# Penguin77jp/RaytracingMin

Measured on AMD Instinct MI355X. Metric: Msamples/s (W*H*spp/s), Cornell box 1080p@1024spp, higher is better.
Workload: dtype f64; 1 GPU; cornellBoxSetting.json rows 0:1080 of 1920x1080 1024spp (SS 4 x S 64), L1 repaired, max_bounces 8, seed 0x5EED, host-libm sin/cos (RTM_MODE_HOST_TRIG), interleaved 8-row bands over 1 GPU(s) + one gather; sample_split_waves_per_tile=8, collective=none (one rank, frame stays in HBM)

## Files before the change

### include/rtm_debug.h

```cpp
#ifndef RTM_DEBUG_H
#define RTM_DEBUG_H

#include "rtm.h"

#ifdef __cplusplus
extern "C" {
#endif

int rtm_debug_math_probe(int op, const double* a, const double* b, size_t n, double* out);
int rtm_debug_trig_table(int entries, double* out);
int rtm_debug_selfcheck(int kind, unsigned long long* mismatches);
int rtm_debug_wf_nearest(int kind, const rtm_sphere* spheres, size_t n, const double* org, const double* dir,
                         size_t n_rays, int32_t* out_id, double* out_t);
int rtm_debug_fp64_peak(int waves_per_simd, double min_ms, double* tflops, double* kernel_ms);
int rtm_debug_grid_nearest(const rtm_sphere* spheres, size_t n, const double* org, const double* dir, size_t n_rays,
                           int32_t* out_id, double* out_t, uint32_t* out_tests, uint32_t* out_steps, uint64_t* info);
int rtm_debug_grid_build(const rtm_sphere* spheres, size_t n, uint64_t* info, double* pads, uint32_t* ranges, size_t ranges_cap,
                         uint32_t* items, size_t items_cap, int32_t* big, size_t big_cap);
int rtm_debug_scene_facts(const rtm_sphere* spheres, size_t n, uint64_t facts[2]);
int rtm_debug_zero_term_facts(const rtm_sphere* spheres, size_t n, uint64_t facts[2]);
int rtm_debug_component_bench(int which, const rtm_sphere* spheres, size_t n, int reps, int blocks, int lds_pad,
                              double* cycles_per_rep);
int rtm_debug_denoise_variance_kernel(int form, const rtm_denoise_var_params* params, int32_t width, int32_t height, int device,
                                      const rtm_aov_buffers* guide_dev, void* work_dev, float* variance_out_dev, void* stream);
int rtm_debug_matte_rank(int32_t super_samples, int32_t layers, int device, const int32_t* ids_dev, size_t n_pixels,
                         int32_t* id_out_dev, float* coverage_out_dev, float* alpha_out_dev, void* stream);

#ifdef __cplusplus
}
#endif
#endif
```

### raytracingmin_amd/_lib.py

```python
import ctypes as C
import os

_HERE = os.path.dirname(os.path.abspath(__file__))
LIB_PATH = os.environ.get("RTM_LIB_OVERRIDE") or os.path.join(_HERE, "librtm_hip.so")

RTM_OK = 0
MODE_LITERAL, MODE_REPAIRED = 0, 1
MODE_HOST_TRIG = 0x100
MODE_COUNT_TESTS = 0x200
MODE_SURFACE_SAMPLE = 0x400
MODES = {"literal": MODE_LITERAL, "repaired": MODE_REPAIRED, 0: 0, 1: 1}


class RtmError(RuntimeError):
    def __init__(self, status, what, detail=""):
        self.status = status
        super().__init__(f"{what}: {detail}" if detail else what)


class rtm_camera(C.Structure):
    _fields_ = [("origin", C.c_double * 3), ("target", C.c_double * 3), ("up", C.c_double * 3),
                ("fov", C.c_float), ("_pad", C.c_float)]


# ... 175 lines not shown
    "rtm_scene_load_json_objects": (C.c_int, [C.c_char_p, C.c_int, _P(rtm_settings), C.c_void_p,
                                              C.c_size_t, _P(C.c_size_t)]),
    "rtm_scene_parse_json_objects": (C.c_int, [C.c_char_p, C.c_size_t, C.c_int, _P(rtm_settings),
                                               C.c_void_p, C.c_size_t, _P(C.c_size_t)]),
    "rtm_scene_save_sample_json": (C.c_int, [C.c_char_p]),
    "rtm_scene_make_stress": (C.c_int, [C.c_uint64, C.c_size_t, _P(rtm_settings), C.c_void_p]),
    "rtm_quantise": (C.c_int, [C.c_void_p, C.c_size_t, C.c_void_p]),
    "rtm_write_bmp": (C.c_int, [C.c_char_p, C.c_int, C.c_int, C.c_int, C.c_void_p]),
    "rtm_write_jpg": (C.c_int, [C.c_char_p, C.c_int, C.c_int, C.c_int, C.c_void_p, C.c_int]),
    "rtm_write_pfm": (C.c_int, [C.c_char_p, C.c_int, C.c_int, C.c_int, C.c_void_p]),
    "rtm_read_pfm": (C.c_int, [C.c_char_p, _P(C.c_int), _P(C.c_int), _P(C.c_int), C.c_void_p, C.c_size_t]),
}
DEBUG_SIGNATURES = {
    "rtm_debug_math_probe": (C.c_int, [C.c_int, C.c_void_p, C.c_void_p, C.c_size_t, C.c_void_p]),
    "rtm_debug_selfcheck": (C.c_int, [C.c_int, C.POINTER(C.c_uint64)]),
    "rtm_debug_trig_table": (C.c_int, [C.c_int, C.c_void_p]),
    "rtm_debug_fp64_peak": (C.c_int, [C.c_int, C.c_double, C.POINTER(C.c_double), C.POINTER(C.c_double)]),
    "rtm_debug_wf_nearest": (C.c_int, [C.c_int, C.c_void_p, C.c_size_t, C.c_void_p, C.c_void_p, C.c_size_t,
                                       C.c_void_p, C.c_void_p]),
    "rtm_debug_grid_nearest": (C.c_int, [C.c_void_p, C.c_size_t, C.c_void_p, C.c_void_p, C.c_size_t, C.c_void_p, C.c_void_p,
                                         C.c_void_p, C.c_void_p, C.c_void_p]),
    "rtm_debug_scene_facts": (C.c_int, [C.c_void_p, C.c_size_t, C.c_void_p]),
    "rtm_debug_zero_term_facts": (C.c_int, [C.c_void_p, C.c_size_t, C.c_void_p]),
    "rtm_debug_grid_build": (C.c_int, [C.c_void_p, C.c_size_t, C.c_void_p, C.c_void_p, C.c_void_p, C.c_size_t, C.c_void_p,
                                       C.c_size_t, C.c_void_p, C.c_size_t]),
    "rtm_debug_denoise_variance_kernel": (C.c_int, [C.c_int, _P(rtm_denoise_var_params), C.c_int32, C.c_int32, C.c_int,
                                                    _P(rtm_aov_buffers), C.c_void_p, C.c_void_p, C.c_void_p]),
    "rtm_debug_matte_rank": (C.c_int, [C.c_int32, C.c_int32, C.c_int, C.c_void_p, C.c_size_t, C.c_void_p, C.c_void_p, C.c_void_p,
                                       C.c_void_p]),
    "rtm_debug_component_bench": (C.c_int, [C.c_int, C.c_void_p, C.c_size_t, C.c_int, C.c_int, C.c_int,
                                            C.POINTER(C.c_double)]),
}
ABI_VERSION = 5

_lib = None


def _share_torch_hip_runtime():
    try:
        import torch
    except ImportError:
        pass


def lib():
    global _lib
# ... 23 lines not shown
```

### raytracingmin_amd/csrc/rtm_api.cpp

```cpp
#include <exception>

#include "../../include/rtm_debug.h"
#include "rtm_internal.h"

#define RTM_GUARD(call)                                  \
    try {                                                \
        return (call);                                   \
    } catch (const std::exception& e) {                  \
        rtm::set_last_error(e.what());                   \
        return RTM_ERR_INVALID_ARGUMENT;                 \
    } catch (...) {                                      \
        rtm::set_last_error("unknown exception");        \
        return RTM_ERR_INVALID_ARGUMENT;                 \
    }

extern "C" {

int rtm_abi_version(void) { return RTM_ABI_VERSION; }

const char* rtm_strerror(int status) {
    switch (status) {
        case RTM_OK: return "ok";
        case RTM_ERR_INVALID_ARGUMENT: return "invalid argument";
        case RTM_ERR_INVALID_SCENE: return "invalid scene";
// ... 166 lines not shown
    RTM_GUARD(rtm::wf_nearest_probe(kind, sp, n, org, dir, n_rays, out_id, out_t))
}
int rtm_debug_denoise_variance_kernel(int form, const rtm_denoise_var_params* params, int32_t width, int32_t height, int device,
                                      const rtm_aov_buffers* guide_dev, void* work_dev, float* variance_out_dev, void* stream) {
    RTM_GUARD(rtm::denoise_variance_kernel_probe(form, params, width, height, device, guide_dev, work_dev, variance_out_dev, stream))
}
int rtm_debug_matte_rank(int32_t super_samples, int32_t layers, int device, const int32_t* ids_dev, size_t n_pixels,
                         int32_t* id_out_dev, float* coverage_out_dev, float* alpha_out_dev, void* stream) {
    RTM_GUARD(rtm::matte_rank_probe(super_samples, layers, device, ids_dev, n_pixels, id_out_dev, coverage_out_dev, alpha_out_dev,
                                    stream))
}
int rtm_debug_trig_table(int entries, double* out) { RTM_GUARD(rtm::trig_table_host(entries, out)) }
int rtm_debug_selfcheck(int kind, unsigned long long* mismatches) { RTM_GUARD(rtm::selfcheck(kind, mismatches)) }
int rtm_debug_grid_nearest(const rtm_sphere* sp, size_t n, const double* org, const double* dir, size_t n_rays,
                           int32_t* out_id, double* out_t, uint32_t* out_tests, uint32_t* out_steps, uint64_t* info) {
    RTM_GUARD(rtm::grid_nearest_probe(sp, n, org, dir, n_rays, out_id, out_t, out_tests, out_steps, info))
}
int rtm_debug_grid_build(const rtm_sphere* sp, size_t n, uint64_t* info, double* pads, uint32_t* ranges, size_t ranges_cap,
                         uint32_t* items, size_t items_cap, int32_t* big, size_t big_cap) {
    RTM_GUARD(rtm::grid_build_host(sp, n, info, pads, ranges, ranges_cap, items, items_cap, big, big_cap))
}
int rtm_debug_scene_facts(const rtm_sphere* sp, size_t n, uint64_t facts[2]) { RTM_GUARD(rtm::scene_facts_host(sp, n, facts)) }
int rtm_debug_zero_term_facts(const rtm_sphere* sp, size_t n, uint64_t facts[2]) { RTM_GUARD(rtm::zero_term_facts_host(sp, n, facts)) }
int rtm_debug_fp64_peak(int waves_per_simd, double min_ms, double* tflops, double* kernel_ms) {
    RTM_GUARD(rtm::fp64_peak(waves_per_simd, min_ms, tflops, kernel_ms))
}

int rtm_scene_load_json(const char* path, int literal_loader, rtm_settings* settings,
                        rtm_sphere* spheres, size_t capacity, size_t* n_spheres) {
    RTM_GUARD(rtm::scene_load_json(path, literal_loader, settings, spheres, capacity, n_spheres))
}
int rtm_scene_parse_json(const char* text, size_t len, int literal_loader, rtm_settings* settings,
                         rtm_sphere* spheres, size_t capacity, size_t* n_spheres) {
    RTM_GUARD(rtm::scene_parse_json(text, len, literal_loader, settings, spheres, capacity, n_spheres))
}
int rtm_scene_save_sample_json(const char* path) { RTM_GUARD(rtm::scene_save_sample_json(path)) }
int rtm_scene_make_stress(uint64_t seed, size_t n, rtm_settings* settings, rtm_sphere* spheres) {
    RTM_GUARD(rtm::scene_make_stress(seed, n, settings, spheres))
}
int rtm_quantise(const double* image, size_t n_values, uint8_t* out) {
    RTM_GUARD(rtm::quantise(image, n_values, out))
}
int rtm_write_bmp(const char* filename, int w, int h, int comp, const void* data) {
    try {
        return rtm::write_bmp(filename, w, h, comp, data);
    } catch (...) {
// ... 27 lines not shown
```

### raytracingmin_amd/csrc/rtm_internal.h

```cpp
#pragma once
#include <stddef.h>
#include <stdint.h>

#include <string>

#include "../../include/rtm.h"

namespace rtm {

void set_last_error(const std::string& s);
const char* last_error();

int device_count(int* count);
int num_variants();
int output_rows(const rtm_options* opt);
int release_scratch(int device);
int stream_release(int device, void* stream);
int wf_nearest_probe(int kind, const rtm_sphere* sp, size_t n, const double* org, const double* dir, size_t n_rays,
                     int32_t* out_id, double* out_t);
const char* variant_name(int v);
int scene_create(const rtm_sphere* sp, size_t n, int on_device, int device, rtm_scene** out);
int scene_create_objects(const rtm_object* objs, size_t n, int device, rtm_scene** out);
int intersect_objects_batch(const rtm_object* objs, const double* org, const double* dir, size_t n, int mode,
                            int32_t* out_hit, double* out_t, double* out_normal);
// ... 47 lines not shown
                  const rtm_options* opt, double* out64, float* out32, uint8_t* out8, void* stream,
                  rtm_stats* stats);
int render_host(const rtm_settings* st, const rtm_sphere* sp, size_t n, const rtm_options* opt,
                double* out64, float* out32, uint8_t* out8, rtm_stats* stats);
int render_host_objects(const rtm_settings* st, const rtm_object* objs, size_t n, const rtm_options* opt,
                        double* out64, float* out32, uint8_t* out8, rtm_stats* stats);
int path_trace_batch(const rtm_sphere* sp, size_t n, const rtm_options* opt, const double* org,
                     const double* dir, size_t n_rays, double* out, uint32_t* out_draws,
                     uint32_t* out_casts);
int surface_sample_batch(const rtm_sphere* sp, size_t n, const rtm_options* opt, const double* org, const double* dir,
                         size_t n_rays, double* out, uint32_t* out_draws, uint32_t* out_casts);
int intersect_batch(const rtm_sphere* sp, const double* org, const double* dir, size_t n, int mode,
                    int32_t* out_hit, double* out_t, double* out_normal);
int rng_batch(uint64_t seed, uint32_t pixel0, uint32_t n_pixels, uint32_t sample, uint32_t n_draws,
              double* out);
double rng_u01_host(uint64_t seed, uint32_t pixel, uint32_t sample, uint32_t index);
int component_bench(int which, const rtm_sphere* sp, size_t n, int reps, int blocks, int lds_pad,
                    double* cycles_per_rep);
int selfcheck(int kind, unsigned long long* mismatches);
int grid_nearest_probe(const rtm_sphere* sp, size_t n, const double* org, const double* dir, size_t n_rays, int32_t* out_id,
                       double* out_t, uint32_t* out_tests, uint32_t* out_steps, uint64_t* info);
int scene_facts_host(const rtm_sphere* sp, size_t n, uint64_t* facts);
int zero_term_facts_host(const rtm_sphere* sp, size_t n, uint64_t* facts);
int grid_build_host(const rtm_sphere* sp, size_t n, uint64_t* info, double* pads, uint32_t* ranges, size_t ranges_cap,
                    uint32_t* items, size_t items_cap, int32_t* big, size_t big_cap);
int fp64_peak(int waves_per_simd, double min_ms, double* tflops, double* kernel_ms);
int math_probe(int op, const double* a, const double* b, size_t n, double* out);
int launch_tol(const void* render_params, size_t params_bytes, unsigned grid, size_t lds_pad, void* stream);
int tol_math_probe(int op, const double* a_dev, const double* b_dev, size_t n, double* out_dev);
int trig_table_host(int entries, double* out);
void release_trig_tab(int device);

int scene_parse_json(const char* text, size_t len, int literal_loader, rtm_settings* st,
                     rtm_sphere* spheres, size_t capacity, size_t* n_spheres);
int scene_parse_json_objects(const char* text, size_t len, int literal_loader, rtm_settings* st,
                             rtm_object* objects, size_t capacity, size_t* n_objects);
int scene_load_json_objects(const char* path, int literal_loader, rtm_settings* st, rtm_object* objects,
                            size_t capacity, size_t* n_objects);
int scene_load_json(const char* path, int literal_loader, rtm_settings* st, rtm_sphere* spheres,
                    size_t capacity, size_t* n_spheres);
int scene_save_sample_json(const char* path);
int scene_make_stress(uint64_t seed, size_t n, rtm_settings* st, rtm_sphere* spheres);
int quantise(const double* image, size_t n_values, uint8_t* out);
int write_bmp(const char* filename, int w, int h, int comp, const void* data);
int write_jpg(const char* filename, int w, int h, int comp, const void* data, int quality);
int write_pfm(const char* filename, int w, int h, int comp, const float* data);
// ... 4 lines not shown
```

### raytracingmin_amd/csrc/rtm_kernels.hip

```cpp
#include <hip/hip_runtime.h>

#include <cfloat>
#include <cmath>
#include <cstdio>
#include <cstdlib>
#include <cstring>
#include <algorithm>
#include <atomic>
#include <thread>
#include <map>
#include <memory>
#include <mutex>
#include <shared_mutex>
#include <tuple>
#include <string>
#include <type_traits>
#include <vector>

#include "../../include/rtm.h"
#include "rtm_device.h"
#include "rtm_host.h"
#include "rtm_path.h"

#include "rtm_render_kernel.h"
// ... 48 lines not shown
        m = m < sp[i].color[2] ? sp[i].color[2] : m;
        const double kd = (double)(float)m;
        mat[i * 8 + 0] = sp[i].color[0] / kd;
        mat[i * 8 + 1] = sp[i].color[1] / kd;
        mat[i * 8 + 2] = sp[i].color[2] / kd;
        mat[i * 8 + 3] = sp[i].emission[0];
        mat[i * 8 + 4] = sp[i].emission[1];
        mat[i * 8 + 5] = sp[i].emission[2];
        mat[i * 8 + 6] = kd;
        mat[i * 8 + 7] = kd * 16777216.0;
    }
}

static uint64_t axis_pattern(const double* geom, size_t n) {
    uint64_t pat = 0;
    for (size_t i = 0; i < n && i < 32; ++i) {
        const double* g = geom + i * 4;
        if (!(std::isfinite(g[0]) && std::isfinite(g[1]) && std::isfinite(g[2])) || !(g[3] >= 0.0)) continue;
        const bool zx = g[0] == 0.0, zy = g[1] == 0.0, zz = g[2] == 0.0;
        const uint64_t a = (!zx && zy && zz) ? 1u : (zx && !zy && zz) ? 2u : (zx && zy && !zz) ? 3u : 0u;
        pat |= a << (2 * i);
    }
    return pat;
}

static unsigned compact_flag_of(const double* geom, size_t n) {
    for (size_t i = 0; i < n; ++i) {
        const double* g = geom + i * 4;
        const double reach = std::sqrt(g[0] * g[0] + g[1] * g[1] + g[2] * g[2]) + std::sqrt(std::fabs(g[3]));
        if (!(reach <= kCompactExtent)) return 0u;
    }
    return kSceneCompact;
}
static unsigned fold_flags_of(const double* mat, size_t n) {
    auto plain = [](double v) { return !std::signbit(v) && !std::isnan(v); };
    for (size_t i = 0; i < n; ++i) {
        const double* m = mat + i * 8;
        if (!(plain(m[3]) && plain(m[4]) && plain(m[5]))) return 0u;
        if (m[6] > 0.0) {
            if (!(m[3] == 0.0 && m[4] == 0.0 && m[5] == 0.0)) return 0u;
            if (!(plain(m[0]) && plain(m[1]) && plain(m[2]))) return 0u;
        }
    }
    return kFoldNoLevelEmission;
}
static unsigned zero_term_flags_of(const double* mat, size_t n, uint64_t* emit_mask) {
// ... 386 lines not shown
            ranges[c * 2] = B.cell_start[c];
            ranges[c * 2 + 1] = B.cell_start[c + 1];
        }
    if (items) std::memcpy(items, B.items.data(), B.refs * sizeof(unsigned));
    if (big && !B.big.empty()) std::memcpy(big, B.big.data(), B.big.size() * sizeof(int));
    return RTM_OK;
}

int scene_facts_host(const rtm_sphere* sp, size_t n, uint64_t* facts) {
    if ((!sp && n) || !facts) return RTM_ERR_INVALID_ARGUMENT;
    std::vector<double> hg, hm;
    flatten_scene(sp, n, hg, hm);
    facts[0] = axis_pattern(hg.data(), n);
    facts[1] = fold_flags_of(hm.data(), n) | compact_flag_of(hg.data(), n);
    return RTM_OK;
}
int zero_term_facts_host(const rtm_sphere* sp, size_t n, uint64_t* facts) {
    if ((!sp && n) || !facts) return RTM_ERR_INVALID_ARGUMENT;
    std::vector<double> hg, hm;
    flatten_scene(sp, n, hg, hm);
    facts[0] = zero_term_flags_of(hm.data(), n, &facts[1]) != 0u ? 1u : 0u;
    return RTM_OK;
}

static int build_scene_grid(rtm_scene& sc, const double* hg, const double* hm, size_t n, int device,
                            const double* plane_rows = nullptr) {
    GridBuild B;
    if (!make_grid(hg, n, B)) return RTM_OK;
    sc.grid_far_bounces = false;
    const double reach = std::sqrt(B.hdr.reach2);
    for (int i : B.big) {
        const bool diffuse = !hm || hm[(size_t)i * 8 + 6] > 0.0;
        if (hg[(size_t)i * 4 + 3] < 0.0) {
            if (!plane_rows) return RTM_OK;
            const double* pl = plane_rows + (size_t)i * 16;
            for (int c = 0; c < 4 && diffuse; ++c) {
                double d2 = 0.0;
                for (int k = 0; k < 3; ++k) {
                    const double p = pl[k] + ((c & 1) ? pl[6 + k] : -pl[6 + k]) + ((c & 2) ? pl[9 + k] : -pl[9 + k]);
                    d2 += (p - B.hdr.cb[k]) * (p - B.hdr.cb[k]);
                }
                if (!(std::sqrt(d2) <= reach)) sc.grid_far_bounces = true;
            }
            continue;
        }
        double d2 = 0.0;
// ... 25 lines not shown
    B.hdr.cell_range = reinterpret_cast<const uint2*>(base + off_cs);
    B.hdr.recs = reinterpret_cast<const double4*>(base + off_items);
    B.hdr.n_recs = (unsigned)B.items.size();
    B.hdr.big = reinterpret_cast<const int*>(base + off_big);
    RTM_HIP_CHECK(hipMemcpy(base, &B.hdr, sizeof B.hdr, hipMemcpyHostToDevice));
    RTM_HIP_CHECK(hipMemcpy(base + off_cs, ranges.data(), ranges.size() * sizeof(unsigned), hipMemcpyHostToDevice));
    RTM_HIP_CHECK(hipMemcpy(base + off_items, recs.data(), recs.size() * sizeof(double), hipMemcpyHostToDevice));
    if (!B.big.empty())
        RTM_HIP_CHECK(hipMemcpy(base + off_big, B.big.data(), B.big.size() * sizeof(int), hipMemcpyHostToDevice));
    sc.grid_hdr = B.hdr;
    sc.grid_cells = B.cell_start.size() - 1;
    sc.grid_refs = B.items.size();
    sc.grid_big = B.big.size();
    return RTM_OK;
}

static int scene_build_host(rtm_scene& sc, const rtm_sphere* sp, size_t n, int device, bool want_grid = true) {
    RTM_HIP_CHECK(hipSetDevice(device));
    sc.device = device;
    sc.n = n;
    std::vector<double> hg, hm, hs;
    flatten_scene(sp, n, hg, hm, &hs);
    sc.axis_pat = axis_pattern(hg.data(), n);
    sc.fold_flags = fold_flags_of(hm.data(), n) | compact_flag_of(hg.data(), n) | zero_term_flags_of(hm.data(), n, &sc.emit_mask);
    int rc = sc.geom.alloc_pooled((n ? n : 1) * 4 * sizeof(double), device);
    if (rc == RTM_OK) rc = sc.mat.alloc_pooled((n + 1) * 8 * sizeof(double), device);
    if (rc == RTM_OK) rc = sc.aux.alloc_pooled(scene_aux_doubles(n) * sizeof(double), device);
    if (rc == RTM_OK) rc = sc.surf.alloc_pooled(hs.size() * sizeof(double), device);
    if (rc != RTM_OK) return rc;
    RTM_HIP_CHECK(hipMemcpy(sc.surf.p, hs.data(), hs.size() * sizeof(double), hipMemcpyHostToDevice));
    if (n) RTM_HIP_CHECK(hipMemcpy(sc.geom.p, hg.data(), hg.size() * sizeof(double), hipMemcpyHostToDevice));
    RTM_HIP_CHECK(hipMemcpy(sc.mat.p, hm.data(), hm.size() * sizeof(double), hipMemcpyHostToDevice));
    rc = launch_scene_aux(sc.geom.as<double>(), n, sc.aux.as<double>(), nullptr);
    if (rc != RTM_OK) return rc;
    RTM_HIP_CHECK(hipStreamSynchronize(nullptr));
    return want_grid ? build_scene_grid(sc, hg.data(), hm.data(), n, device) : RTM_OK;
}
static int scene_build_device(rtm_scene& sc, const rtm_sphere* sp_dev, size_t n, int device) {
    RTM_HIP_CHECK(hipSetDevice(device));
    sc.device = device;
    sc.n = n;
    int rc = sc.geom.alloc_pooled((n ? n : 1) * 4 * sizeof(double), device);
    if (rc == RTM_OK) rc = sc.mat.alloc_pooled((n + 1) * 8 * sizeof(double), device);
    if (rc == RTM_OK) rc = sc.aux.alloc_pooled(scene_aux_doubles(n) * sizeof(double), device);
    if (rc == RTM_OK) rc = sc.surf.alloc_pooled((n ? n : 1) * 4 * sizeof(double), device);
    if (rc != RTM_OK) return rc;
    flatten_scene_kernel<<<(unsigned)((n + 1 + 255) / 256), 256>>>(sp_dev, n, sc.geom.as<double>(), sc.mat.as<double>(), sc.surf.as<double>());
    RTM_HIP_CHECK(hipGetLastError());
    rc = launch_scene_aux(sc.geom.as<double>(), n, sc.aux.as<double>(), nullptr);
    if (rc != RTM_OK) return rc;
    RTM_HIP_CHECK(hipStreamSynchronize(nullptr));
    if (n > 0 && n <= 32) {
        std::vector<double> rows(n * 4);
        RTM_HIP_CHECK(hipMemcpy(rows.data(), sc.geom.p, rows.size() * sizeof(double), hipMemcpyDeviceToHost));
        sc.axis_pat = axis_pattern(rows.data(), n);
        std::vector<double> mrows((n + 1) * 8);
        RTM_HIP_CHECK(hipMemcpy(mrows.data(), sc.mat.p, mrows.size() * sizeof(double), hipMemcpyDeviceToHost));
        sc.fold_flags = fold_flags_of(mrows.data(), n) | compact_flag_of(rows.data(), n) | zero_term_flags_of(mrows.data(), n, &sc.emit_mask);
    }
    if (n < kGridMinSpheres) return RTM_OK;
    std::vector<double> hg(n * 4);
    RTM_HIP_CHECK(hipMemcpy(hg.data(), sc.geom.p, hg.size() * sizeof(double), hipMemcpyDeviceToHost));
    std::vector<double> hm((n + 1) * 8);
    RTM_HIP_CHECK(hipMemcpy(hm.data(), sc.mat.p, hm.size() * sizeof(double), hipMemcpyDeviceToHost));
    return build_scene_grid(sc, hg.data(), hm.data(), n, device);
}

int scene_create(const rtm_sphere* sp, size_t n, int on_device, int device, rtm_scene** out) {
    if (!out || (!sp && n) || n > 0x7FFFFFFFull) return invalid("null argument or scene too large");
    *out = nullptr;
    std::unique_ptr<rtm_scene> sc(new rtm_scene);
    const int rc = on_device ? scene_build_device(*sc, sp, n, device) : scene_build_host(*sc, sp, n, device);
    if (rc != RTM_OK) return rc;
    *out = sc.release();
    return RTM_OK;
}
static void plane_row(const rtm_object& o, double row[16]) {
    using namespace host;
    const H3 pos = {o.position[0], o.position[1], o.position[2]};
    const H3 nrm = normalize(sub(H3{o.target[0], o.target[1], o.target[2]}, pos));
    const H3 rn = normalize(cross(nrm, H3{o.up[0], o.up[1], o.up[2]}));
// ... 2004 lines not shown
```

### raytracingmin_amd/csrc/rtm_kernels_tol.hip

```cpp
#define RTM_NS rtm_tol
#define RTM_TOL 1
#include <hip/hip_runtime.h>

#include <cmath>
#include <cstdlib>
#include <cstring>
#include <map>
#include <mutex>
#include <vector>

#include "rtm_internal.h"
#include "rtm_render_kernel.h"

namespace rtm_tol {

static bool compact_launch(const RenderParams& P) {
    const double cam = std::sqrt(P.cam_org.x * P.cam_org.x + P.cam_org.y * P.cam_org.y + P.cam_org.z * P.cam_org.z);
    return (P.scene.fold_flags & kSceneCompact) != 0u && cam <= kCompactExtent;
}

constexpr unsigned kTolCapped = kLdsTab | kPark | kPack8 | kDefer | kSteal;
constexpr unsigned kTolAny = kLdsTab | kPark | kDefer | kPackL;
constexpr int kTolWavesPerSimd = 4;

template <unsigned F>
static void launch_n(const RenderParams& P, unsigned grid, size_t lds_pad, hipStream_t stream) {
    constexpr int LDS_D = (F & kPackL) != 0 ? 0 : 16;
    unsigned unit_tab;
    render_lds_bytes<F, uint8_t, LDS_D>(P.scene.n, lds_pad, &unit_tab);
    const bool axis = P.mode == RTM_MODE_REPAIRED && unit_tab == 1u && compact_launch(P);
#define RTM_AXIS_CASE(k, sig)                                                                                    \
    if (P.scene.n == k && P.scene.axis_pat == sig && axis) {                                                     \
        launch_tiles<MathFast, F, axis_unroll(k, sig), uint8_t, LDS_D, kTolWavesPerSimd>(P, grid, lds_pad, stream); \
        return;                                                                                                  \
    }
    if constexpr ((F & kPackL) != 0) {
        RTM_AXIS_CASE(7, kAxisSigCornell7)
    } else {
        RTM_AXIS_SIGNATURES(RTM_AXIS_CASE)
        switch (P.scene.n) {
            case 3: launch_tiles<MathFast, F, -103, uint8_t, LDS_D, kTolWavesPerSimd>(P, grid, lds_pad, stream); return;
            case 5: launch_tiles<MathFast, F, -105, uint8_t, LDS_D, kTolWavesPerSimd>(P, grid, lds_pad, stream); return;
            case 7: launch_tiles<MathFast, F, -107, uint8_t, LDS_D, kTolWavesPerSimd>(P, grid, lds_pad, stream); return;
            default: break;
        }
    }
#undef RTM_AXIS_CASE
    if (P.scene.n < 8) launch_tiles<MathFast, F, -8, uint8_t, LDS_D, kTolWavesPerSimd>(P, grid, lds_pad, stream);
    else launch_tiles<MathFast, F, 8, uint8_t, LDS_D, kTolWavesPerSimd>(P, grid, lds_pad, stream);
}

template <unsigned F>
static void launch_row(const RenderParams& P, unsigned grid, size_t lds_pad, hipStream_t stream) {
    if (P.split > 1) {
        launch_n<F | kSplit>(P, P.split_first + P.n_tiles * P.split, lds_pad, stream);
        launch_split_finalize(P, stream);
    } else {
        launch_n<F>(P, grid, lds_pad, stream);
    }
    if constexpr ((F & kSteal) != 0) launch_steal_finalize(P, grid, stream);
}

__global__ void tol_math_probe_kernel(int op, const double* __restrict__ a, const double* __restrict__ b, size_t n,
                                      double* __restrict__ out, const double2* __restrict__ tab) {
    const size_t i = (size_t)blockIdx.x * blockDim.x + threadIdx.x;
    if (i >= n) return;
    const double x = a[i], y = b ? b[i] : 0.0;
    double r = 0.0, s, c;
    switch (op) {
        case 32: r = seq_sqrt(x); break;
        case 33: r = seq_quot(x, y, seq_rcp(y)); break;
        case 34: r = seq_rcp(x); break;
        case 35: r = x * y + 1.0; break;
        case 36: sincos_small(x, s, c); r = s; break;
        case 37: sincos_small(x, s, c); r = c; break;
        case 38: r = fold_step(d3(x, x, x), d3(y, y, y), d3(0.25, 0.25, 0.25)).y; break;
        case 39: sincos_turn24_k(TrigFromRegs{}, x, s, c); r = s; break;
        case 40: sincos_turn24_k(TrigFromRegs{}, x, s, c); r = c; break;
        case 41: {
            const double in[1] = {x};
            double out1[1];
            seq_sqrt_batch<1, true>(in, out1);
            r = out1[0];
            break;
        }
        case 42: sincos_turn24_tab_apply(sincos_turn24_tab_load(tab, (uint32_t)x), s, c); r = s; break;
        case 43: sincos_turn24_tab_apply(sincos_turn24_tab_load(tab, (uint32_t)x), s, c); r = c; break;
        case 44: { MathSpec m; r = m.sqrt64_unit(x); } break;
        case 45: {
// ... 147 lines not shown
```

### raytracingmin_amd/csrc/rtm_path.h

```cpp
#pragma once
#include <cfloat>
#include <type_traits>

#include "../../include/rtm.h"
#include "rtm_device.h"

namespace RTM_NS {


__device__ __forceinline__ double seq_rcp(const double y) {
    double r = __builtin_amdgcn_rcp(y);
    double e = __builtin_fma(-y, r, 1.0);
#if RTM_TOL
    return __builtin_fma(r, __builtin_fma(e, e, e), r);
#else
    r = __builtin_fma(r, e, r);
    e = __builtin_fma(-y, r, 1.0);
    return __builtin_fma(r, e, r);
#endif
}
__device__ __forceinline__ double seq_quot(const double x, const double y, const double r) {
#if RTM_TOL
    (void)y;
    return x * r;
// ... 439 lines not shown
    const double4* recs;
    const int* big;
};

struct SceneView {
    const double4* __restrict__ geom;
    const double* __restrict__ mat;
    int n;
    const double* __restrict__ wprime = nullptr;
    const double* __restrict__ bounds = nullptr;
    const float4* __restrict__ geom32 = nullptr;
    const float4* __restrict__ geom32s = nullptr;
    const uint32_t* __restrict__ trig_fix = nullptr;
    const double* __restrict__ plane = nullptr;
    const GridHeader* __restrict__ grid = nullptr;
    const double* __restrict__ surf = nullptr;
    unsigned long long axis_pat = 0ull;
    unsigned fold_flags = 0u;
    unsigned long long emit_mask = ~0ull;
};
constexpr unsigned kFoldNoLevelEmission = 1u;
constexpr unsigned kFoldZeroTermSkippable = 4u;
constexpr unsigned kSceneCompact = 2u;
constexpr double kCompactExtent = 1e7;

__device__ __forceinline__ bool plane_test(const double* __restrict__ pl, const D3 org, const D3 dir, double& t) {
    const D3 pos = d3(pl[0], pl[1], pl[2]), nrm = d3(pl[3], pl[4], pl[5]);
    const double dn = dot(nrm, dir);
    if (fabs(dn) < (double)FLT_EPSILON) return false;
    const double tt = dot(nrm, pos - org) / dn;
    if (!(tt > 0.001)) return false;
    const D3 d = (org + dir * tt) - pos;
    const D3 right = d3(pl[6], pl[7], pl[8]), upv = d3(pl[9], pl[10], pl[11]);
    if (fabs(dot(d, right)) > pl[12] || fabs(dot(d, upv)) > pl[13]) return false;
    t = tt;
    return true;
}

struct TrigFixWord {
    uint32_t word;
    int off;
};
__device__ __forceinline__ TrigFixWord trig_fix_load(const uint32_t* __restrict__ fix, const RngStream& rng) {
    const uint32_t k = mix32((rng.ctr - 2u * 0x9E3779B9u) ^ rng.k1) >> 9;
    return TrigFixWord{fix[k >> 3], (int)(k & 7u) * 4};
}
// ... 165 lines not shown
                best = m;
            }
            dis = best;
            hit_object = (int)((((uint32_t)__double2loint(best)) + 1u) & 7u) - 1;
            return;
        }
    }
    if (!PACKID && far == 0ull) {
#pragma unroll
        for (int k = 0; k < K; ++k) {
            const unsigned long long accept = __builtin_amdgcn_ballot_w64(t1v[k] < dis);
            hit_object = sel_index_mask(accept, i0 + k, hit_object);
            double m;
            asm("v_min_f64 %0, %1, %2" : "=v"(m) : "v"(dis), "v"(t1v[k]));
            dis = m;
        }
        return;
    }
#endif
#pragma unroll
    for (int k = 0; k < K; ++k) accept_update(b[k], sq[k], i0 + k, dis, hit_object);
}

struct AxisShared {
#if RTM_TOL
    double Pyz, Pxz, Pxy, Qyz, Qxz, Qxy;
#else
    double Px, Py, Pz, Pxy, Qx, Qy, Qz, Qxy;
#endif
    __device__ __forceinline__ AxisShared(const D3 org, const D3 dir) {
        const double px = org.x * dir.x, py = org.y * dir.y, pz = org.z * dir.z;
        const double qx = org.x * org.x, qy = org.y * org.y, qz = org.z * org.z;
#if RTM_TOL
        Pyz = py + pz; Pxz = px + pz; Pxy = px + py;
        Qyz = qy + qz; Qxz = qx + qz; Qxy = qx + qy;
#else
        Px = px; Py = py; Pz = pz; Pxy = px + py;
        Qx = qx; Qy = qy; Qz = qz; Qxy = qx + qy;
#endif
    }
};
constexpr unsigned kAxisSigCornell7 = 2u | (1u << 2) | (1u << 4) | (2u << 6) | (2u << 8) | (3u << 10) | (3u << 12);
constexpr unsigned kAxisSigSimple5 = (1u << 2) | (1u << 4) | (2u << 6) | (2u << 8);
constexpr unsigned kAxisSigSetting3 = 2u | (1u << 4);
constexpr int axis_unroll(const int n, const unsigned sig) { return -(1000 + n + 8 * (int)sig); }
#define RTM_AXIS_SIGNATURES(X) X(7, kAxisSigCornell7) X(5, kAxisSigSimple5) X(3, kAxisSigSetting3)
__device__ __forceinline__ void sphere_disc(const double4 g, const unsigned pat, const D3 org, const D3 dir,
                                            const AxisShared& A, double& b, double& D4) {
    if (pat == 1u) {
        const double px = g.x - org.x;
#if RTM_TOL
        b = px * dir.x - A.Pyz;
        D4 = b * b - (px * px + A.Qyz) + g.w;
#else
        b = px * dir.x - A.Py - A.Pz;
        D4 = b * b - (px * px + A.Qy + A.Qz) + g.w;
#endif
    } else if (pat == 2u) {
        const double py = g.y - org.y;
#if RTM_TOL
        b = py * dir.y - A.Pxz;
        D4 = b * b - (py * py + A.Qxz) + g.w;
#else
        b = py * dir.y - A.Px - A.Pz;
        D4 = b * b - (A.Qx + py * py + A.Qz) + g.w;
#endif
    } else if (pat == 3u) {
        const double pz = g.z - org.z;
        b = pz * dir.z - A.Pxy;
        D4 = b * b - (A.Qxy + pz * pz) + g.w;
    } else {
        const D3 p_o = d3(g.x - org.x, g.y - org.y, g.z - org.z);
        b = dot(p_o, dir);
        D4 = b * b - dot(p_o, p_o) + g.w;
    }
}

template <class M, int K, bool EARLY_OUT = false>
__device__ __forceinline__ void sphere_chunk_g(const double4 (&g)[K], const int i0, const D3 org, const D3 dir,
                                               double& dis, int& hit_object) {
    double b[K], D4[K], sq[K];
#pragma unroll
    for (int k = 0; k < K; ++k) {
        const D3 p_o = d3(g[k].x - org.x, g[k].y - org.y, g[k].z - org.z);
        b[k] = dot(p_o, dir);
        D4[k] = b[k] * b[k] - dot(p_o, p_o) + g[k].w;
    }
    if constexpr (EARLY_OUT) {
        double top = D4[0];
#pragma unroll
        for (int k = 1; k < K; ++k) top = __builtin_fmax(top, D4[k]);
        if (__builtin_amdgcn_ballot_w64(top >= 0.0) == 0) return;
#pragma unroll
        for (int k = 0; k < K; ++k) {
            if (__builtin_amdgcn_ballot_w64(D4[k] >= 0.0) == 0) continue;
            const double sqk = M::sqrt64(D4[k]);
            const double t1 = b[k] - sqk, t2 = b[k] + sqk;
            const double t = (t1 > 0.001) ? t1 : t2;
            const bool accept = (t < dis) && !(t < (double)1e-5f);
            dis = accept ? t : dis;
            hit_object = accept ? i0 + k : hit_object;
        }
        return;
    }
    M::template sqrt64_batch_hit<K>(D4, sq);
#pragma unroll
    for (int k = 0; k < K; ++k) accept_update(b[k], sq[k], i0 + k, dis, hit_object);
}
constexpr int kGeomPhase = 2;
template <class M, int K, class Scene, bool EARLY_OUT = false, unsigned SIG = 0u>
__device__ __forceinline__ void sphere_chunk(const Scene& sc, const int i0, const D3 org, const D3 dir,
                                             double& dis, int& hit_object) {
    static_assert(SIG == 0u || (K > kGeomPhase && K < 8 && !EARLY_OUT), "an axis signature names the spheres of ONE exact chunk");
    constexpr int PH = kGeomPhase;
    if constexpr (K > PH && !EARLY_OUT) {
        double b[K], D4[K], sq[K];
        if constexpr (SIG != 0u) {
            const AxisShared A(org, dir);
            constexpr int PA = 2;
#pragma unroll
            for (int k0 = 0; k0 < K; k0 += PA) {
                double4 g[PA];
#pragma unroll
                for (int k = 0; k < PA; ++k)
                    if (k0 + k < K) g[k] = sc.geom_uniform(i0 + k0 + k);
#pragma unroll
                for (int k = 0; k < PA; ++k)
                    if (k0 + k < K) sphere_disc(g[k], (SIG >> (2 * (k0 + k))) & 3u, org, dir, A, b[k0 + k], D4[k0 + k]);
                __builtin_amdgcn_sched_barrier(0);
            }
            M::template sqrt64_batch_hit<K, RTM_TOL != 0>(D4, sq);
            accept_batch<K, RTM_TOL != 0>(b, sq, i0, dis, hit_object);
            return;
        }
#pragma unroll
        for (int k0 = 0; k0 < K; k0 += PH) {
            double4 g[PH];
#pragma unroll
            for (int k = 0; k < PH; ++k)
                if (k0 + k < K) g[k] = sc.geom_uniform(i0 + k0 + k);
#pragma unroll
            for (int k = 0; k < PH; ++k)
                if (k0 + k < K) {
                    const D3 p_o = d3(g[k].x - org.x, g[k].y - org.y, g[k].z - org.z);
                    b[k0 + k] = dot(p_o, dir);
                    D4[k0 + k] = b[k0 + k] * b[k0 + k] - dot(p_o, p_o) + g[k].w;
                }
            __builtin_amdgcn_sched_barrier(0);
        }
        if constexpr (K >= 8)
            M::template sqrt64_batch<K>(D4, sq);
// ... 826 lines not shown
```

Measured before the change: 22060 Msamples/s.

## Precompute expanded axis-sphere rows and share constant term across Cornell walls

For axis-aligned giant spheres (the Cornell walls), the intersection discriminant is rewritten in expanded form using per-sphere precomputed rows (c, -2c, c^2-r^2) stored after the geometry array. Per ray it computes o·d and o·o once. Walls that share an identical constant term reuse one o·o+K value. A new specialised launch case for the 7-sphere Cornell signature with a shared-K mask is added, guarded by a host-side error bound that checks the expanded form stays within tolerance. This is meant to cut FP64 adds and multiplies in the inner intersection loop, at the cost of extra scalar loads and a stricter precision-based eligibility check.

```diff
diff --git a/include/rtm_debug.h b/include/rtm_debug.h
--- a/include/rtm_debug.h
+++ b/include/rtm_debug.h
@@ -19,6 +19,7 @@
                          uint32_t* items, size_t items_cap, int32_t* big, size_t big_cap);
 int rtm_debug_scene_facts(const rtm_sphere* spheres, size_t n, uint64_t facts[2]);
 int rtm_debug_zero_term_facts(const rtm_sphere* spheres, size_t n, uint64_t facts[2]);
+int rtm_debug_axis_rows(const rtm_sphere* spheres, size_t n, double* rows);
 int rtm_debug_component_bench(int which, const rtm_sphere* spheres, size_t n, int reps, int blocks, int lds_pad,
                               double* cycles_per_rep);
 int rtm_debug_denoise_variance_kernel(int form, const rtm_denoise_var_params* params, int32_t width, int32_t height, int device,
diff --git a/raytracingmin_amd/_lib.py b/raytracingmin_amd/_lib.py
--- a/raytracingmin_amd/_lib.py
+++ b/raytracingmin_amd/_lib.py
@@ -221,6 +221,7 @@
                                          C.c_void_p, C.c_void_p, C.c_void_p]),
     "rtm_debug_scene_facts": (C.c_int, [C.c_void_p, C.c_size_t, C.c_void_p]),
     "rtm_debug_zero_term_facts": (C.c_int, [C.c_void_p, C.c_size_t, C.c_void_p]),
+    "rtm_debug_axis_rows": (C.c_int, [C.c_void_p, C.c_size_t, C.c_void_p]),
     "rtm_debug_grid_build": (C.c_int, [C.c_void_p, C.c_size_t, C.c_void_p, C.c_void_p, C.c_void_p, C.c_size_t, C.c_void_p,
                                        C.c_size_t, C.c_void_p, C.c_size_t]),
     "rtm_debug_denoise_variance_kernel": (C.c_int, [C.c_int, _P(rtm_denoise_var_params), C.c_int32, C.c_int32, C.c_int,
diff --git a/raytracingmin_amd/csrc/rtm_api.cpp b/raytracingmin_amd/csrc/rtm_api.cpp
--- a/raytracingmin_amd/csrc/rtm_api.cpp
+++ b/raytracingmin_amd/csrc/rtm_api.cpp
@@ -212,6 +212,7 @@
 }
 int rtm_debug_scene_facts(const rtm_sphere* sp, size_t n, uint64_t facts[2]) { RTM_GUARD(rtm::scene_facts_host(sp, n, facts)) }
 int rtm_debug_zero_term_facts(const rtm_sphere* sp, size_t n, uint64_t facts[2]) { RTM_GUARD(rtm::zero_term_facts_host(sp, n, facts)) }
+int rtm_debug_axis_rows(const rtm_sphere* sp, size_t n, double* rows) { RTM_GUARD(rtm::axis_rows_host(sp, n, rows)) }
 int rtm_debug_fp64_peak(int waves_per_simd, double min_ms, double* tflops, double* kernel_ms) {
     RTM_GUARD(rtm::fp64_peak(waves_per_simd, min_ms, tflops, kernel_ms))
 }
diff --git a/raytracingmin_amd/csrc/rtm_internal.h b/raytracingmin_amd/csrc/rtm_internal.h
--- a/raytracingmin_amd/csrc/rtm_internal.h
+++ b/raytracingmin_amd/csrc/rtm_internal.h
@@ -93,6 +93,7 @@
                        double* out_t, uint32_t* out_tests, uint32_t* out_steps, uint64_t* info);
 int scene_facts_host(const rtm_sphere* sp, size_t n, uint64_t* facts);
 int zero_term_facts_host(const rtm_sphere* sp, size_t n, uint64_t* facts);
+int axis_rows_host(const rtm_sphere* sp, size_t n, double* rows);
 int grid_build_host(const rtm_sphere* sp, size_t n, uint64_t* info, double* pads, uint32_t* ranges, size_t ranges_cap,
                     uint32_t* items, size_t items_cap, int32_t* big, size_t big_cap);
 int fp64_peak(int waves_per_simd, double min_ms, double* tflops, double* kernel_ms);
diff --git a/raytracingmin_amd/csrc/rtm_kernels.hip b/raytracingmin_amd/csrc/rtm_kernels.hip
--- a/raytracingmin_amd/csrc/rtm_kernels.hip
+++ b/raytracingmin_amd/csrc/rtm_kernels.hip
@@ -94,6 +94,69 @@
         pat |= a << (2 * i);
     }
     return pat;
+}
+constexpr size_t kAxisRowsMax = 32;
+static size_t axis_row_count(size_t n) { return n <= kAxisRowsMax ? n : 0; }
+static double axis_q_err(double own_reach, double reach) {
+    const double m = own_reach > reach ? own_reach : reach;
+    return std::ldexp(m * m, -49);
+}
+static bool axis_self_hit_safe(double c, double r2) {
+    const double r = std::sqrt(r2), own = std::fabs(c) + r;
+    return r > 0.0 && std::isfinite(own) && axis_q_err(own, 0.0) / (2.0 * r) <= std::ldexp((double)1e-5f, -17);
+}
+static unsigned axis_reach_bits(const double* geom, size_t n, uint64_t pat) {
+    if (axis_row_count(n) == 0 || pat == 0) return 0u;
+    double extent = 0.0, reach = kCompactExtent;
+    for (size_t i = 0; i < n; ++i) {
+        const double* g = geom + i * 4;
+        const double own = std::sqrt(g[0] * g[0] + g[1] * g[1] + g[2] * g[2]) + std::sqrt(std::fabs(g[3]));
+        if (!std::isfinite(own)) return 0u;
+        extent = own > extent ? own : extent;
+        const unsigned a = (unsigned)(pat >> (2 * i)) & 3u;
+        if (a == 0u) continue;
+        if (!axis_self_hit_safe(g[a - 1u], g[3])) return 0u;
+        const double rho = std::sqrt(std::ldexp((double)1e-5f * std::sqrt(g[3]), 46));
+        reach = rho < reach ? rho : reach;
+    }
+    const int k = std::ilogb(reach);
+    if (!(reach >= 1.0) || !(extent <= std::ldexp(1.0, k))) return 0u;
+    return (unsigned)(128 + k) << kSceneAxisReachShift;
+}
+static void axis_rows(const double* geom, size_t n, uint64_t pat, double* rows) {
+    const unsigned e = (axis_reach_bits(geom, n, pat) >> kSceneAxisReachShift) & kSceneAxisReachMask;
+    const double reach = e ? std::ldexp(1.0, (int)e - 128) : 0.0;
+    for (size_t i = 0; i < axis_row_count(n); ++i) {
+        const unsigned a = (unsigned)(pat >> (2 * i)) & 3u;
+        double* row = rows + i * 4;
+        row[0] = row[1] = row[2] = row[3] = 0.0;
+        if (a == 0u) continue;
+        const double c = geom[i * 4 + (a - 1u)];
+        row[0] = c;
+        row[1] = -2.0 * c;
+        row[2] = (double)fmal((long double)c, (long double)c, -(long double)geom[i * 4 + 3]);
+        row[3] = reach;
+    }
+}
+static unsigned shared_k_bits(const double* geom, size_t n, uint64_t pat) {
+    if (axis_row_count(n) == 0) return 0u;
+    std::vector<double> rows(n * 4);
+    axis_rows(geom, n, pat, rows.data());
+    unsigned best = 0u, best_count = 1u;
+    for (size_t i = 0; i < n && i < 8; ++i) {
+        if (((pat >> (2 * i)) & 3u) == 0u) continue;
+        unsigned mask = 0u, count = 0u;
+        for (size_t j = i; j < n && j < 8; ++j)
+            if (((pat >> (2 * j)) & 3u) != 0u && std::memcmp(&rows[j * 4 + 2], &rows[i * 4 + 2], sizeof(double)) == 0) {
+                mask |= 1u << j;
+                ++count;
+            }
+        if (count > best_count) {
+            best = mask;
+            best_count = count;
+        }
+    }
+    return best << kSceneSharedKShift;
 }
 
 static unsigned compact_flag_of(const double* geom, size_t n) {
@@ -526,6 +589,13 @@
     facts[0] = zero_term_flags_of(hm.data(), n, &facts[1]) != 0u ? 1u : 0u;
     return RTM_OK;
 }
+int axis_rows_host(const rtm_sphere* sp, size_t n, double* rows) {
+    if ((!sp && n) || !rows || n > kAxisRowsMax) return RTM_ERR_INVALID_ARGUMENT;
+    std::vector<double> hg, hm;
+    flatten_scene(sp, n, hg, hm);
+    axis_rows(hg.data(), n, axis_pattern(hg.data(), n), rows);
+    return RTM_OK;
+}
 
 static int build_scene_grid(rtm_scene& sc, const double* hg, const double* hm, size_t n, int device,
                             const double* plane_rows = nullptr) {
@@ -597,8 +667,11 @@
     std::vector<double> hg, hm, hs;
     flatten_scene(sp, n, hg, hm, &hs);
     sc.axis_pat = axis_pattern(hg.data(), n);
-    sc.fold_flags = fold_flags_of(hm.data(), n) | compact_flag_of(hg.data(), n) | zero_term_flags_of(hm.data(), n, &sc.emit_mask);
-    int rc = sc.geom.alloc_pooled((n ? n : 1) * 4 * sizeof(double), device);
+    sc.fold_flags = fold_flags_of(hm.data(), n) | compact_flag_of(hg.data(), n) | zero_term_flags_of(hm.data(), n, &sc.emit_mask) |
+                    shared_k_bits(hg.data(), n, sc.axis_pat) | axis_reach_bits(hg.data(), n, sc.axis_pat);
+    hg.resize((n + axis_row_count(n)) * 4);
+    axis_rows(hg.data(), n, sc.axis_pat, hg.data() + n * 4);
+    int rc = sc.geom.alloc_pooled((hg.empty() ? 1 : hg.size() / 4) * 4 * sizeof(double), device);
     if (rc == RTM_OK) rc = sc.mat.alloc_pooled((n + 1) * 8 * sizeof(double), device);
     if (rc == RTM_OK) rc = sc.aux.alloc_pooled(scene_aux_doubles(n) * sizeof(double), device);
     if (rc == RTM_OK) rc = sc.surf.alloc_pooled(hs.size() * sizeof(double), device);
@@ -615,7 +688,7 @@
     RTM_HIP_CHECK(hipSetDevice(device));
     sc.device = device;
     sc.n = n;
-    int rc = sc.geom.alloc_pooled((n ? n : 1) * 4 * sizeof(double), device);
+    int rc = sc.geom.alloc_pooled((n ? n + axis_row_count(n) : 1) * 4 * sizeof(double), device);
     if (rc == RTM_OK) rc = sc.mat.alloc_pooled((n + 1) * 8 * sizeof(double), device);
     if (rc == RTM_OK) rc = sc.aux.alloc_pooled(scene_aux_doubles(n) * sizeof(double), device);
     if (rc == RTM_OK) rc = sc.surf.alloc_pooled((n ? n : 1) * 4 * sizeof(double), device);
@@ -629,9 +702,13 @@
         std::vector<double> rows(n * 4);
         RTM_HIP_CHECK(hipMemcpy(rows.data(), sc.geom.p, rows.size() * sizeof(double), hipMemcpyDeviceToHost));
         sc.axis_pat = axis_pattern(rows.data(), n);
+        std::vector<double> arows(n * 4);
+        axis_rows(rows.data(), n, sc.axis_pat, arows.data());
+        RTM_HIP_CHECK(hipMemcpy(sc.geom.as<double>() + n * 4, arows.data(), arows.size() * sizeof(double), hipMemcpyHostToDevice));
         std::vector<double> mrows((n + 1) * 8);
         RTM_HIP_CHECK(hipMemcpy(mrows.data(), sc.mat.p, mrows.size() * sizeof(double), hipMemcpyDeviceToHost));
-        sc.fold_flags = fold_flags_of(mrows.data(), n) | compact_flag_of(rows.data(), n) | zero_term_flags_of(mrows.data(), n, &sc.emit_mask);
+        sc.fold_flags = fold_flags_of(mrows.data(), n) | compact_flag_of(rows.data(), n) | zero_term_flags_of(mrows.data(), n, &sc.emit_mask) |
+                        shared_k_bits(rows.data(), n, sc.axis_pat) | axis_reach_bits(rows.data(), n, sc.axis_pat);
     }
     if (n < kGridMinSpheres) return RTM_OK;
     std::vector<double> hg(n * 4);
diff --git a/raytracingmin_amd/csrc/rtm_kernels_tol.hip b/raytracingmin_amd/csrc/rtm_kernels_tol.hip
--- a/raytracingmin_amd/csrc/rtm_kernels_tol.hip
+++ b/raytracingmin_amd/csrc/rtm_kernels_tol.hip
@@ -18,6 +18,11 @@
     const double cam = std::sqrt(P.cam_org.x * P.cam_org.x + P.cam_org.y * P.cam_org.y + P.cam_org.z * P.cam_org.z);
     return (P.scene.fold_flags & kSceneCompact) != 0u && cam <= kCompactExtent;
 }
+static bool expanded_form_launch(const RenderParams& P) {
+    const unsigned e = (P.scene.fold_flags >> kSceneAxisReachShift) & kSceneAxisReachMask;
+    const double cam = std::sqrt(P.cam_org.x * P.cam_org.x + P.cam_org.y * P.cam_org.y + P.cam_org.z * P.cam_org.z);
+    return e != 0u && cam <= std::ldexp(1.0, (int)e - 128);
+}
 
 constexpr unsigned kTolCapped = kLdsTab | kPark | kPack8 | kDefer | kSteal;
 constexpr unsigned kTolAny = kLdsTab | kPark | kDefer | kPackL;
@@ -28,7 +33,15 @@
     constexpr int LDS_D = (F & kPackL) != 0 ? 0 : 16;
     unsigned unit_tab;
     render_lds_bytes<F, uint8_t, LDS_D>(P.scene.n, lds_pad, &unit_tab);
-    const bool axis = P.mode == RTM_MODE_REPAIRED && unit_tab == 1u && compact_launch(P);
+    const bool axis = P.mode == RTM_MODE_REPAIRED && unit_tab == 1u && compact_launch(P) && expanded_form_launch(P);
+    const unsigned shared_k = (P.scene.fold_flags >> kSceneSharedKShift) & kSceneSharedKMask;
+#define RTM_AXIS_CASE(k, sig)                                                                                    \
+    if (P.scene.n == k && P.scene.axis_pat == ((sig) & 0xFFFFu) && shared_k == ((sig) >> kAxisSharedKShift) && axis) { \
+        launch_tiles<MathFast, F, axis_unroll(k, sig), uint8_t, LDS_D, kTolWavesPerSimd>(P, grid, lds_pad, stream); \
+        return;                                                                                                  \
+    }
+    RTM_AXIS_CASE(7, kAxisSigCornell7Walls)
+#undef RTM_AXIS_CASE
 #define RTM_AXIS_CASE(k, sig)                                                                                    \
     if (P.scene.n == k && P.scene.axis_pat == sig && axis) {                                                     \
         launch_tiles<MathFast, F, axis_unroll(k, sig), uint8_t, LDS_D, kTolWavesPerSimd>(P, grid, lds_pad, stream); \
@@ -65,6 +78,26 @@
                                       double* __restrict__ out, const double2* __restrict__ tab) {
     const size_t i = (size_t)blockIdx.x * blockDim.x + threadIdx.x;
     if (i >= n) return;
+    if (op >= 52 && op <= 54) {
+        const size_t j = i & ~(size_t)7;
+        double bb = 0.0, D4 = 0.0;
+        if (b && j + 7 < n) {
+            const D3 org = d3(a[j], a[j + 1], a[j + 2]), dir = d3(a[j + 3], a[j + 4], a[j + 5]);
+            const unsigned pat = (unsigned)b[j];
+            const double c = b[j + 1];
+            if (pat >= 1u && pat <= 3u) {
+                if (op == 52) {
+                    const double4 g = double4{pat == 1u ? c : 0.0, pat == 2u ? c : 0.0, pat == 3u ? c : 0.0, b[j + 2]};
+                    sphere_disc_ref(g, pat, org, dir, AxisSharedRef(org, dir), bb, D4);
+                } else {
+                    const AxisShared A(org, dir);
+                    sphere_disc(double4{}, AxisRow{c, b[j + 3], b[j + 4]}, pat, op == 54, A.oo + b[j + 4], org, dir, A, bb, D4);
+                }
+            }
+        }
+        out[i] = (i & 7) == 0 ? bb : (i & 7) == 1 ? D4 : 0.0;
+        return;
+    }
     const double x = a[i], y = b ? b[i] : 0.0;
     double r = 0.0, s, c;
     switch (op) {
diff --git a/raytracingmin_amd/csrc/rtm_path.h b/raytracingmin_amd/csrc/rtm_path.h
--- a/raytracingmin_amd/csrc/rtm_path.h
+++ b/raytracingmin_amd/csrc/rtm_path.h
@@ -485,6 +485,8 @@
 constexpr unsigned kFoldNoLevelEmission = 1u;
 constexpr unsigned kFoldZeroTermSkippable = 4u;
 constexpr unsigned kSceneCompact = 2u;
+constexpr unsigned kSceneSharedKShift = 8u, kSceneSharedKMask = 0xFFu;
+constexpr unsigned kSceneAxisReachShift = 16u, kSceneAxisReachMask = 0xFFu;
 constexpr double kCompactExtent = 1e7;
 
 __device__ __forceinline__ bool plane_test(const double* __restrict__ pl, const D3 org, const D3 dir, double& t) {
@@ -696,49 +698,76 @@
     for (int k = 0; k < K; ++k) accept_update(b[k], sq[k], i0 + k, dis, hit_object);
 }
 
+#if RTM_TOL
+struct AxisRow {
+    double c, m2c, K;
+};
+__device__ __forceinline__ AxisRow load_axis_row_uniform(const double4* geom, int i) {
+#if defined(__HIP_DEVICE_COMPILE__)
+    typedef const __attribute__((address_space(4))) double* ConstF64Ptr;
+    ConstF64Ptr p = (ConstF64Ptr)(unsigned long long)(geom + i);
+    return AxisRow{p[0], p[1], p[2]};
+#else
+    return AxisRow{geom[i].x, geom[i].y, geom[i].z};
+#endif
+}
 struct AxisShared {
-#if RTM_TOL
+    double od, oo;
+    __device__ __forceinline__ AxisShared(const D3 org, const D3 dir) : od(dot(org, dir)), oo(dot(org, org)) {}
+};
+struct AxisSharedRef {
     double Pyz, Pxz, Pxy, Qyz, Qxz, Qxy;
-#else
+    __device__ __forceinline__ AxisSharedRef(const D3 org, const D3 dir) {
+        const double px = org.x * dir.x, py = org.y * dir.y, pz = org.z * dir.z;
+        const double qx = org.x * org.x, qy = org.y * org.y, qz = org.z * org.z;
+        Pyz = py + pz; Pxz = px + pz; Pxy = px + py;
+        Qyz = qy + qz; Qxz = qx + qz; Qxy = qx + qy;
+    }
+};
+#else
+struct AxisShared {
     double Px, Py, Pz, Pxy, Qx, Qy, Qz, Qxy;
-#endif
     __device__ __forceinline__ AxisShared(const D3 org, const D3 dir) {
         const double px = org.x * dir.x, py = org.y * dir.y, pz = org.z * dir.z;
         const double qx = org.x * org.x, qy = org.y * org.y, qz = org.z * org.z;
-#if RTM_TOL
-        Pyz = py + pz; Pxz = px + pz; Pxy = px + py;
-        Qyz = qy + qz; Qxz = qx + qz; Qxy = qx + qy;
-#else
         Px = px; Py = py; Pz = pz; Pxy = px + py;
         Qx = qx; Qy = qy; Qz = qz; Qxy = qx + qy;
-#endif
     }
 };
+#endif
 constexpr unsigned kAxisSigCornell7 = 2u | (1u << 2) | (1u << 4) | (2u << 6) | (2u << 8) | (3u << 10) | (3u << 12);
 constexpr unsigned kAxisSigSimple5 = (1u << 2) | (1u << 4) | (2u << 6) | (2u << 8);
 constexpr unsigned kAxisSigSetting3 = 2u | (1u << 4);
 constexpr int axis_unroll(const int n, const unsigned sig) { return -(1000 + n + 8 * (int)sig); }
+constexpr unsigned kAxisSharedKShift = 16u;
+constexpr unsigned kAxisSigCornell7Walls = kAxisSigCornell7 | (0x7Eu << kAxisSharedKShift);
 #define RTM_AXIS_SIGNATURES(X) X(7, kAxisSigCornell7) X(5, kAxisSigSimple5) X(3, kAxisSigSetting3)
-__device__ __forceinline__ void sphere_disc(const double4 g, const unsigned pat, const D3 org, const D3 dir,
-                                            const AxisShared& A, double& b, double& D4) {
+#if RTM_TOL
+__device__ __forceinline__ void sphere_disc(const double4 g, const AxisRow r, const unsigned pat, const bool shared_k,
+                                            const double ooK, const D3 org, const D3 dir, const AxisShared& A, double& b,
+                                            double& D4) {
+    if (pat != 0u) {
+        const double oa = pat == 1u ? org.x : pat == 2u ? org.y : org.z;
+        const double da = pat == 1u ? dir.x : pat == 2u ? dir.y : dir.z;
+        b = r.c * da - A.od;
+        const double c = shared_k ? r.m2c * oa + ooK : r.m2c * oa + A.oo + r.K;
+        D4 = b * b - c;
+    } else {
+        const D3 p_o = d3(g.x - org.x, g.y - org.y, g.z - org.z);
+        b = dot(p_o, dir);
+        D4 = b * b - dot(p_o, p_o) + g.w;
+    }
+}
+__device__ __forceinline__ void sphere_disc_ref(const double4 g, const unsigned pat, const D3 org, const D3 dir,
+                                                const AxisSharedRef& A, double& b, double& D4) {
     if (pat == 1u) {
         const double px = g.x - org.x;
-#if RTM_TOL
         b = px * dir.x - A.Pyz;
         D4 = b * b - (px * px + A.Qyz) + g.w;
-#else
-        b = px * dir.x - A.Py - A.Pz;
-        D4 = b * b - (px * px + A.Qy + A.Qz) + g.w;
-#endif
     } else if (pat == 2u) {
         const double py = g.y - org.y;
-#if RTM_TOL
         b = py * dir.y - A.Pxz;
         D4 = b * b - (py * py + A.Qxz) + g.w;
-#else
-        b = py * dir.y - A.Px - A.Pz;
-        D4 = b * b - (A.Qx + py * py + A.Qz) + g.w;
-#endif
     } else if (pat == 3u) {
         const double pz = g.z - org.z;
         b = pz * dir.z - A.Pxy;
@@ -749,6 +778,28 @@
         D4 = b * b - dot(p_o, p_o) + g.w;
     }
 }
+#else
+__device__ __forceinline__ void sphere_disc(const double4 g, const unsigned pat, const D3 org, const D3 dir,
+                                            const AxisShared& A, double& b, double& D4) {
+    if (pat == 1u) {
+        const double px = g.x - org.x;
+        b = px * dir.x - A.Py - A.Pz;
+        D4 = b * b - (px * px + A.Qy + A.Qz) + g.w;
+    } else if (pat == 2u) {
+        const double py = g.y - org.y;
+        b = py * dir.y - A.Px - A.Pz;
+        D4 = b * b - (A.Qx + py * py + A.Qz) + g.w;
+    } else if (pat == 3u) {
+        const double pz = g.z - org.z;
+        b = pz * dir.z - A.Pxy;
+        D4 = b * b - (A.Qxy + pz * pz) + g.w;
+    } else {
+        const D3 p_o = d3(g.x - org.x, g.y - org.y, g.z - org.z);
+        b = dot(p_o, dir);
+        D4 = b * b - dot(p_o, p_o) + g.w;
+    }
+}
+#endif
 
 template <class M, int K, bool EARLY_OUT = false>
 __device__ __forceinline__ void sphere_chunk_g(const double4 (&g)[K], const int i0, const D3 org, const D3 dir,
@@ -791,9 +842,30 @@
         double b[K], D4[K], sq[K];
         if constexpr (SIG != 0u) {
             const AxisShared A(org, dir);
+#if RTM_TOL
+            double ooK = 0.0;
+#endif
             constexpr int PA = 2;
 #pragma unroll
             for (int k0 = 0; k0 < K; k0 += PA) {
+#if RTM_TOL
+                constexpr unsigned KM = SIG >> kAxisSharedKShift;
+                double4 g[PA] = {};
+                AxisRow r[PA] = {};
+#pragma unroll
+                for (int k = 0; k < PA; ++k)
+                    if (k0 + k < K) {
+                        if (((SIG >> (2 * (k0 + k))) & 3u) != 0u) r[k] = load_axis_row_uniform(sc.v.geom, K + i0 + k0 + k);
+                        else g[k] = sc.geom_uniform(i0 + k0 + k);
+                    }
+#pragma unroll
+                for (int k = 0; k < PA; ++k)
+                    if (k0 + k < K) {
+                        const bool shared_k = ((KM >> (k0 + k)) & 1u) != 0u;
+                        if (shared_k && (KM & ((1u << (k0 + k)) - 1u)) == 0u) ooK = A.oo + r[k].K;
+                        sphere_disc(g[k], r[k], (SIG >> (2 * (k0 + k))) & 3u, shared_k, ooK, org, dir, A, b[k0 + k], D4[k0 + k]);
+                    }
+#else
                 double4 g[PA];
 #pragma unroll
                 for (int k = 0; k < PA; ++k)
@@ -801,6 +873,7 @@
 #pragma unroll
                 for (int k = 0; k < PA; ++k)
                     if (k0 + k < K) sphere_disc(g[k], (SIG >> (2 * (k0 + k))) & 3u, org, dir, A, b[k0 + k], D4[k0 + k]);
+#endif
                 __builtin_amdgcn_sched_barrier(0);
             }
             M::template sqrt64_batch_hit<K, RTM_TOL != 0>(D4, sq);
```

After: 22910 Msamples/s, median of 6. 3.9% higher.
